# Ryannasr11/m2-tts

Hardware: AMD Instinct MI355X
Metric: audio samples/sec (22.05 kHz) + RTF, stage1_poc batch=32 @1/2/4/8 MI355X (higher is better)
Workload: dtype f32 (split 3xf16 MFMA, fp32 accumulate); 1 GPU; stage1_poc SimpleVocoder B=32 per GPU (configs[1]); stage=s1, per_gpu_batch=32, mel_frames=500, audio_samples_per_utt=32000, parallelism=weak-scaled replicas x1 (dp1, no collective in the data path)

## Files before the change

m2-tts_amd/csrc/m2_common.h:

```cpp
#pragma once

#include <hip/hip_runtime.h>
#include <stdint.h>
#include <string>

#include "../../include/m2tts_hip.h"

namespace m2 {

constexpr int kWave = 64;
constexpr float kLnEps = 1e-5f;
constexpr float kLeaky = 0.1f;
constexpr float kMaskFill = -1e9f;

enum Act : int { ACT_NONE = 0, ACT_LEAKY = 1, ACT_TANH = 2, ACT_RELU = 3, ACT_SOFTPLUS = 4 };

void set_error(const std::string& msg);

struct Switches {
    int dur_rb = 0;
    int dur_count = -1;
    int speculative = 1;
    bool tf_chain = true;
    bool tf_layer = true;
    bool tf_unfused = false;
    int tf_waves = 0;
    int tfl_rb = 0;
    int tfl_first_rb = 0;
    int tfl_rb_masked = 0;
    int tfl_rb_unmasked = 0;
    int tfl_qs2 = -1;
    int att_qt = 0;
    bool att_f32 = false;
    bool voc_perlayer = false;
    bool voc_f32 = false;
    bool voc_tail_x3 = false;
    bool voc_mid_x3 = false;
    int voc_plan = -1;
    int f32_mt = 2;
    bool f32_pair = true;
    int x3_head_prio = 0;
    bool f32_comp = true;
    int midp_nch = 0;
    int tailp_nch = 0;
    bool tailp_seven = false;
    int tailp2_nch = 0;
    bool tailp2_seven = false;
    bool head_inconv = false;
    int s2_mid_alt = -1;
    int s2_head_tf = 0;
    int redo_grid = -1;
    bool redo_launch = false;
    bool dur_split = true;
    bool dur_pers = true;
};
const Switches& sw();
void reload_switches();

int32_t fail(int32_t code, const char* what);
int32_t hip_status(hipError_t e, const char* where);

#define M2_CHECK_ARG(cond, msg)                      \
    do {                                             \
        if (!(cond)) return ::m2::fail(M2_E_ARG, msg); \
    } while (0)
#define M2_CHECK_SHAPE(cond, msg)                      \
    do {                                               \
        if (!(cond)) return ::m2::fail(M2_E_SHAPE, msg); \
    } while (0)
#define M2_HIP(expr)                                                   \
    do {                                                               \
        hipError_t _e = (expr);                                        \
        if (_e != hipSuccess) return ::m2::hip_status(_e, #expr);      \
    } while (0)
#define M2_LAUNCHED(name)                                              \
    do {                                                               \
        hipError_t _e = hipGetLastError();                             \
        if (_e != hipSuccess) return ::m2::hip_status(_e, name);       \
    } while (0)

__device__ __forceinline__ float apply_act(float v, int act) {
    if (act == ACT_LEAKY) return v > 0.f ? v : v * kLeaky;
    if (act == ACT_TANH) return tanhf(v);
    if (act == ACT_RELU) return v > 0.f ? v : 0.f;
    if (act == ACT_SOFTPLUS) return v > 20.f ? v : log1pf(expf(v));
    return v;
}

template <int ACT>
__device__ __forceinline__ float act_t(float v) {
    if constexpr (ACT == ACT_LEAKY) return fmaxf(v, v * kLeaky);
    else if constexpr (ACT == ACT_TANH) return tanhf(v);
    else if constexpr (ACT == ACT_RELU) return v > 0.f ? v : 0.f;
    else return v;
}

__device__ __forceinline__ int dev_frames(const int32_t* p, int cap) {
    const int t = max(1, *p);
    return t <= cap ? t : 0;
}

inline int cdiv(int a, int b) { return (a + b - 1) / b; }
inline size_t align_up(size_t v, size_t a) { return (v + a - 1) / a * a; }

struct Carve {
    char* base;
    size_t cap;
    size_t off = 0;
    bool ok = true;
    Carve(void* p, size_t n) : base(static_cast<char*>(p)), cap(n) {}
    template <typename T>
    T* take(size_t count) {
        size_t o = align_up(off, 256);
        size_t n = count * sizeof(T);
        if (o + n > cap || base == nullptr) { ok = false; off = o + n; return nullptr; }
        off = o + n;
        return reinterpret_cast<T*>(base + o);
    }
};

struct Sizer {
    size_t off = 0;
    template <typename T>
    T* take(size_t count) { off = align_up(off, 256) + count * sizeof(T); return nullptr; }
};

__device__ __forceinline__ void ln_row_stats(const float* xr, int K, int lane, float& mean, float& rstd) {
    float s = 0.f;
    for (int k = lane; k < K; k += 64) s = __fadd_rn(s, xr[k]);
    for (int o = 32; o > 0; o >>= 1) s = __fadd_rn(s, __shfl_xor(s, o));
    mean = __fdiv_rn(s, (float)K);
    float v = 0.f;
    for (int k = lane; k < K; k += 64) {
        const float d = __fsub_rn(xr[k], mean);
        v = __fmaf_rn(d, d, v);
    }
    for (int o = 32; o > 0; o >>= 1) v = __fadd_rn(v, __shfl_xor(v, o));
    rstd = __fdiv_rn(1.0f, __fsqrt_rn(__fadd_rn(__fdiv_rn(v, (float)K), kLnEps)));
}

template <int KP>
__device__ __forceinline__ void ln_row_stats_regs(const float (&x)[KP], int K, int lane, float& mean, float& rstd) {
    float s = 0.f;
#pragma unroll
    for (int q = 0; q < KP; ++q)
        if (lane + 64 * q < K) s = __fadd_rn(s, x[q]);
    for (int o = 32; o > 0; o >>= 1) s = __fadd_rn(s, __shfl_xor(s, o));
    mean = __fdiv_rn(s, (float)K);
    float v = 0.f;
#pragma unroll
    for (int q = 0; q < KP; ++q)
        if (lane + 64 * q < K) {
            const float d = __fsub_rn(x[q], mean);
            v = __fmaf_rn(d, d, v);
        }
    for (int o = 32; o > 0; o >>= 1) v = __fadd_rn(v, __shfl_xor(v, o));
    rstd = __fdiv_rn(1.0f, __fsqrt_rn(__fadd_rn(__fdiv_rn(v, (float)K), kLnEps)));
}

__device__ __forceinline__ float ln_apply(float x, float mean, float rstd, float g, float b) {
    return __fmaf_rn(__fmul_rn(__fsub_rn(x, mean), rstd), g, b);
}

}
```

m2-tts_amd/csrc/m2_runtime.hip:

```cpp
#include <immintrin.h>

#include <atomic>
#include <climits>
#include <cmath>
#include <cstdlib>
#include <cstring>
#include <mutex>
#include <new>
#include <string>
#include <vector>

#include "m2_common.h"
#include "m2_model.h"
#include "transformer_fused.h"
#include "transformer_layer.h"
#include "vocoder_fused.h"

namespace m2 {

namespace {
std::atomic<const Switches*> g_swp{nullptr};
std::mutex g_sw_mu;
int env_int(const char* name, int dflt) {
    const char* e = std::getenv(name);
    return (e && *e) ? std::atoi(e) : dflt;
}
bool env_set(const char* name) { return std::getenv(name) != nullptr; }
bool env_on(const char* name, bool dflt) {
    const char* e = std::getenv(name);
    return (e && *e) ? std::atoi(e) != 0 : dflt;
}
const bool g_sw_loaded = (reload_switches(), true);
}

const Switches& sw() { return *g_swp.load(std::memory_order_acquire); }

void reload_switches() {
    void* raw = std::calloc(1, sizeof(Switches));
    if (!raw) return;
    Switches& s = *new (raw) Switches();
    const int rb = env_int("M2_DUR_RB", 0);
    s.dur_rb = (rb == 1 || rb == 2) ? rb : 0;
    s.dur_count = std::getenv("M2_DUR_COUNT") && *std::getenv("M2_DUR_COUNT") ? (env_int("M2_DUR_COUNT", 0) != 0) : -1;
    s.speculative = env_on("M2_SPECULATIVE", true) ? 1 : 0;
    s.tf_chain = env_on("M2_TF_CHAIN", true);
    s.tf_layer = env_on("M2_TF_LAYER", true);
    s.tf_unfused = env_set("M2_TF_UNFUSED");
    const int tw = env_int("M2_TF_WAVES", 0);
    s.tf_waves = (tw == 4 || tw == 8) ? tw : 0;
    auto rb124 = [](int v) { return (v == 1 || v == 2 || v == 4) ? v : 0; };
    const int trb = env_int("M2_TFL_RB", 0);
    s.tfl_rb = rb124(trb);
    s.tfl_first_rb = rb124(env_int("M2_TFL_FIRST_RB", 0));
    s.tfl_rb_masked = rb124(env_int("M2_TFL_RB_MASKED", 0));
    s.tfl_rb_unmasked = rb124(env_int("M2_TFL_RB_UNMASKED", 0));
    if (const char* e = std::getenv("M2_TFL_QS2"); e && *e) {
        const int v = std::atoi(e);
        s.tfl_qs2 = (v == 2 || v == 3 || v == 4 || v == 12) ? v : 0;
    }
    s.att_qt = env_int("M2_ATT_QT", 0);
    if (const char* e = std::getenv("M2_ATT_F32")) s.att_f32 = *e && *e != '0';
    s.voc_perlayer = env_set("M2_VOCODER_PERLAYER");
    s.voc_f32 = env_set("M2_VOC_F32");
    s.voc_tail_x3 = env_set("M2_VOC_TAIL_X3");
    s.voc_mid_x3 = env_set("M2_VOC_MID_X3");
    s.voc_plan = env_int("M2_VOC_PLAN", -1);
    s.f32_mt = env_int("M2_F32_MT", 2);
    s.f32_pair = env_int("M2_F32_PAIR", 1) != 0;
    s.f32_comp = env_int("M2_F32_COMP", 1) != 0;
    s.x3_head_prio = env_int("M2_X3_HEAD_PRIO", 0);
    const int mn = env_int("M2_MIDP_NCH", 0);
    s.midp_nch = mn > 0 ? mn : 0;
    const int tn = env_int("M2_TAILP_NCH", 0);
    s.tailp_nch = tn > 0 ? tn : 0;
    s.tailp_seven = env_set("M2_TAILP_SEVEN");
    s.tailp2_nch = env_int("M2_TAILP2_NCH", 0);
    s.tailp2_seven = env_set("M2_TAILP2_SEVEN");
    s.head_inconv = env_set("M2_HEAD_INCONV");
    const int malt = env_int("M2_S2_MID_ALT", -1);
    s.s2_mid_alt = (malt == 0 || malt == 1) ? malt : -1;
    const int htf = env_int("M2_S2_HEAD_TF", env_set("M2_S2_HEAD_TF16") ? 16 : 0);
    s.s2_head_tf = (htf == 16 || htf == 19 || htf == 24 || htf == 27) ? htf : 0;
    s.redo_grid = env_int("M2_REDO_GRID", -1);
    s.redo_launch = env_set("M2_REDO_LAUNCH");
    s.dur_split = env_on("M2_DUR_SPLIT", true);
    s.dur_pers = env_on("M2_DUR_PERS", true);
    std::lock_guard<std::mutex> lk(g_sw_mu);
    const Switches* cur = g_swp.load(std::memory_order_relaxed);
    if (cur && std::memcmp(cur, &s, sizeof(Switches)) == 0) {
        std::free(raw);
        return;
    }
    g_swp.store(&s, std::memory_order_release);
}

int32_t launch_embed_pe(const int64_t*, const float*, const float*, int, int, int, int, float*, const int64_t*,
                        uint8_t*, hipStream_t);
int32_t launch_layer_norm(const float*, const float*, const float*, int, int, float*, hipStream_t);
int32_t launch_linear(const float*, const float*, const float*, const float*, const float*,
                      const float*, int, int, int, int, float*, hipStream_t);
int32_t launch_attention(const float*, const uint8_t*, int, int, int, int, float*, hipStream_t, bool force_f32 = false);
int32_t launch_duration(const float*, int, int, int, const float* const*, float*, hipStream_t,
                        const float* ln_g = nullptr, const float* ln_b = nullptr, float* enc_out = nullptr,
                        const float* const* wsplit = nullptr);
int32_t launch_duration_count(const float*, int, int, int, const float* const*, float*, hipStream_t, const float*,
                              const float*, float*, float, int32_t*, int32_t*, int32_t*, unsigned*, int32_t*, int32_t,
                              const float* const* wsplit = nullptr);
bool duration_count_fusable(int, int);
int32_t launch_lr_count(const void*, int, float, int, int, int32_t*, int32_t*, int32_t*, hipStream_t);
int32_t launch_lr_count_sync(const void*, int, float, int, int, int32_t*, int32_t*, int32_t*, unsigned*, int32_t*,
                             int32_t, hipStream_t);
int32_t launch_lr_expand(const float*, const int32_t*, int, int, int, int, float*, hipStream_t);
int32_t launch_conv(const float*, const float*, const float*, const float*, const float*,
                    const float*, int, int, bool, int, int, int, int, float*, hipStream_t);
int32_t launch_add_pe(const float*, const float*, int, int, int, float*, hipStream_t);
int32_t launch_embed_pe_scaled(const int64_t*, const float*, const float*, int, int, int, int, float, float*, hipStream_t);
int32_t launch_convT(const float*, const float*, const float*, int, int, int, int, int, int,
                     float*, hipStream_t);
int32_t launch_conv_general(const float*, const float*, const float*, const float*, const float*, const float*, int,
                            int, int, int, int, int, int, int, float*, hipStream_t);
int32_t launch_ragged_count(const int32_t*, int, int32_t*, hipStream_t);
int32_t launch_ragged_zero(float*, const int32_t*, int, int, int, hipStream_t);
int32_t launch_ragged_tail(const VocRedoW*, int, int, const float*, bool, const int32_t*, int, int, float*, hipStream_t);
int ragged_window_frames();
int32_t launch_ragged_gather(const float*, bool, const int32_t*, int, int, int, float*, hipStream_t);
int32_t launch_ragged_scatter(const float*, const int32_t*, int, int, float*, hipStream_t);

static thread_local std::string g_last_error;

void set_error(const std::string& msg) { g_last_error = msg; }

int32_t fail(int32_t code, const char* what) {
    set_error(what);
    return code;
}

int32_t hip_status(hipError_t e, const char* where) {
    set_error(std::string(where) + ": " + hipGetErrorString(e));
    return static_cast<int32_t>(e);
}

static constexpr int kVocHalo = 3;
static constexpr int32_t kMaxFrames = 1 << 24;

}

using namespace m2;

namespace {

int32_t mask_kernel_launch(const int64_t* lengths, int B, int S, uint8_t* mask, hipStream_t st);

__global__ void padding_mask_kernel(const int64_t* __restrict__ lengths, int B, int S,
                                    uint8_t* __restrict__ mask) {
    const int i = blockIdx.x * blockDim.x + threadIdx.x;
    if (i >= B * S) return;
    const int b = i / S, s = i - b * S;
    mask[i] = (int64_t)s < lengths[b] ? 1 : 0;
}

int32_t mask_kernel_launch(const int64_t* lengths, int B, int S, uint8_t* mask, hipStream_t st) {
    if (B * S == 0) return M2_OK;
    hipLaunchKernelGGL(padding_mask_kernel, dim3(cdiv(B * S, 256)), dim3(256), 0, st, lengths, B, S, mask);
    M2_LAUNCHED("padding_mask_kernel");
    return M2_OK;
}

struct TfBufs {
    float *x, *qkv, *att, *hid;
    uint8_t* mask;
    TflBufs tfl[2];
};

template <typename A>
void carve_tf(A& a, int B, int N, int H, int heads, TfBufs* out) {
    const size_t R = (size_t)B * N;
    float* x = a.template take<float>(R * H);
    uint8_t* mask = a.template take<uint8_t>(R);
    const size_t three = align_up(R * 3 * H * 4, 256) + align_up(R * H * 4, 256) + align_up(R * 2 * H * 4, 256);
    const size_t one = tfl_supported(H, heads) ? 2 * align_up(tfl_bytes(B, N, H, heads), 256) : 0;
    unsigned char* region = a.template take<unsigned char>(std::max(three, one));
    if (!out) return;
    *out = TfBufs{};
    out->x = x;
    out->mask = mask;
    if (!region) return;
    out->qkv = reinterpret_cast<float*>(region);
    out->att = reinterpret_cast<float*>(region + align_up(R * 3 * H * 4, 256));
    out->hid = reinterpret_cast<float*>(region + align_up(R * 3 * H * 4, 256) + align_up(R * H * 4, 256));
    if (one) {
        tfl_carve(region, B, N, H, heads, &out->tfl[0]);
        tfl_carve(region + align_up(tfl_bytes(B, N, H, heads), 256), B, N, H, heads, &out->tfl[1]);
    }
}

size_t vocoder_max_cl(const m2_config& c, int T) {
    size_t best = (size_t)c.vocoder_channels * T;
    size_t ch = c.vocoder_channels, L = T;
    for (int k = 0; k < 4; ++k) {
        ch /= 2;
        L *= kRates[k];
        best = std::max(best, ch * L);
    }
    return best;
}

template <typename A>
void carve_voc(A& a, const m2_config& c, int B, int T, float** bufs) {
    const size_t n = (size_t)B * vocoder_max_cl(c, T);
    for (int i = 0; i < 3; ++i) {
        float* p = a.template take<float>(n);
        if (bufs) bufs[i] = p;
    }
}

struct ChunkBufs {
    float *mel, *audio, *voc[3];
};

template <typename A>
void carve_chunked(A& a, const m2_config& c, int B, int T, int chunk, ChunkBufs* out) {
    const int W = std::min(T, chunk + 2 * kVocHalo);
    float* mel = a.template take<float>((size_t)B * c.mel_channels * W);
    float* audio = a.template take<float>((size_t)B * 64 * W);
    float* voc[3];
    carve_voc(a, c, B, W, voc);
    if (out) *out = ChunkBufs{mel, audio, {voc[0], voc[1], voc[2]}};
}

size_t vocoder_ws_bytes(const m2_model* m, int B, int T) {
    Sizer s;
    if (m->chunk_frames > 0 && T > m->chunk_frames) carve_chunked(s, m->cfg, B, T, m->chunk_frames, nullptr);
    else carve_voc(s, m->cfg, B, T, nullptr);
    return s.off;
}

struct FrontBufs {
    float *enc, *dur;
    int32_t *cum, *tot, *tmax;
    uint8_t* mask;
};

template <typename A>
void carve_front(A& a, int B, int S, int H, FrontBufs* out) {
    float* enc = a.template take<float>((size_t)B * S * H);
    float* dur = a.template take<float>((size_t)B * S);
    int32_t* cum = a.template take<int32_t>((size_t)B * (S + 1));
    int32_t* tot = a.template take<int32_t>((size_t)B);
    int32_t* tmax = a.template take<int32_t>(1);
    uint8_t* mask = a.template take<uint8_t>((size_t)B * S);
    if (out) *out = FrontBufs{enc, dur, cum, tot, tmax, mask};
}

int32_t run_layer(const m2_model* m, const m2_layer_w& L, const float* x_in, float* x, TfBufs& wb,
                  const uint8_t* mask, int B, int N, hipStream_t st) {
    const int H = m->cfg.hidden_dim, R = B * N;
    int32_t rc;
    if (m->tfused) {
        if ((rc = launch_ln_gemm(x_in, L.n1_w, L.n1_b, L.qkv_p, nullptr, ACT_NONE, R, H, 3 * H, wb.qkv, st))) return rc;
        if ((rc = launch_attention(wb.qkv, mask, B, N, H, m->cfg.num_heads, wb.att, st, m->att_f32))) return rc;
        return launch_post_attn(wb.att, x_in, L.out_p, L.out_b, L.n2_w, L.n2_b, L.ff1_p, L.ff1_b, L.ff2_p, L.ff2_b, R, H,
                                x, st);
    }
    if ((rc = launch_linear(x_in, L.n1_w, L.n1_b, L.qkv_w, nullptr, nullptr, ACT_NONE, R, H, 3 * H, wb.qkv, st))) return rc;
    if ((rc = launch_attention(wb.qkv, mask, B, N, H, m->cfg.num_heads, wb.att, st, m->att_f32))) return rc;
    if ((rc = launch_linear(wb.att, nullptr, nullptr, L.out_w, L.out_b, x_in, ACT_NONE, R, H, H, x, st))) return rc;
    if ((rc = launch_linear(x, L.n2_w, L.n2_b, L.ff1_w, L.ff1_b, nullptr, ACT_RELU, R, H, 2 * H, wb.hid, st))) return rc;
    if ((rc = launch_linear(wb.hid, nullptr, nullptr, L.ff2_w, L.ff2_b, x, ACT_NONE, R, 2 * H, H, x, st))) return rc;
    return M2_OK;
}

bool tf_chain(const m2_model* m) {
    const int H = m->cfg.hidden_dim;
    return sw().tf_chain && m->tfused && tf_post_next_supported(H, 3 * H);
}

bool tf_first_fused(const m2_model* m, const std::vector<m2_layer_w>& layers) {
    return tf_chain(m) && !layers.empty() && tf_src_fused_supported(m->cfg.hidden_dim, 3 * m->cfg.hidden_dim);
}

TflQueue tfl_queue(const m2_model* m) { return TflQueue{m->tflq, m->tfl_seq++}; }
int32_t tfl_reset(const m2_model* m, hipStream_t st, int32_t rc) {
    (void)hipMemsetAsync(m->tflq, 0, kTflQueueWords * sizeof(unsigned), st);
    m->tfl_seq = 0;
    return rc;
}

bool tfl_use(const m2_model* m, const std::vector<m2_layer_w>& layers) {
    return sw().tf_layer && m->tfused && !m->att_f32 && !layers.empty() &&
           tfl_supported(m->cfg.hidden_dim, m->cfg.num_heads);
}

int32_t run_tfl(const m2_model* m, const std::vector<m2_layer_w>& layers, const float* x0, float* x, TfBufs& wb,
                const int64_t* lengths, int B, int N, hipStream_t st, const float* fin_g = nullptr,
                const float* fin_b = nullptr, const float* fin_W = nullptr, const float* fin_bias = nullptr,
                int fin_N = 0, float* fin_out = nullptr, bool* fin_done = nullptr, const int32_t* dN = nullptr,
                const int32_t* rows = nullptr) {
    const int H = m->cfg.hidden_dim, heads = m->cfg.num_heads, n = (int)layers.size();
    if (fin_done) *fin_done = false;
    const float* cur = x0;
    for (int l = 0; l < n; ++l) {
        const m2_layer_w& L = layers[l];
        TflLayer w{L.out_p, L.out_b, L.n2_w, L.n2_b, L.ff1_p, L.ff1_b, L.ff2_p, L.ff2_b};
        w.wide_scores = L.wide_scores;
        int next = 0, NN = 0;
        float* z = nullptr;
        if (l + 1 < n) {
            next = 1;
            w.gn = layers[l + 1].n1_w;
            w.bn = layers[l + 1].n1_b;
            w.Wn = layers[l + 1].qkv_p;
        } else if (fin_W && tfl_proj_supported(H, fin_N)) {
            next = 2;
            w.gn = fin_g;
            w.bn = fin_b;
            w.Wn = fin_W;
            w.bn2 = fin_bias;
            NN = fin_N;
            z = fin_out;
        }
        const int32_t rc = launch_tfl_layer(w, B, N, H, heads, lengths != nullptr, lengths, cur, x, wb.tfl[l & 1], next,
                                            wb.tfl[(l + 1) & 1], NN, z, tfl_queue(m), st, dN, rows);
        if (rc) return tfl_reset(m, st, rc);
        if (next == 2 && fin_done) *fin_done = true;
        cur = x;
    }
    return M2_OK;
}

int32_t run_stack(const m2_model* m, const std::vector<m2_layer_w>& layers, const float* x_in, float* x, TfBufs& wb,
                  const uint8_t* mask, int B, int N, hipStream_t st, const float* fin_g = nullptr,
                  const float* fin_b = nullptr, const float* fin_W = nullptr, const float* fin_bias = nullptr,
                  int fin_N = 0, float* fin_out = nullptr, bool* fin_done = nullptr, bool qkv_ready = false) {
    const int H = m->cfg.hidden_dim, R = B * N, n = (int)layers.size();
    if (fin_done) *fin_done = false;
    int32_t rc;
    const bool chain = tf_chain(m);
    if (!chain) {
        const float* cur = x_in;
        for (const auto& L : layers) {
            if ((rc = run_layer(m, L, cur, x, wb, mask, B, N, st))) return rc;
            cur = x;
        }
        return M2_OK;
    }
    if (n == 0) return M2_OK;
    const float* cur = x_in;
    if (!qkv_ready && (rc = launch_ln_gemm(cur, layers[0].n1_w, layers[0].n1_b, layers[0].qkv_p, nullptr, ACT_NONE, R,
                                           H, 3 * H, wb.qkv, st)))
        return rc;
    for (int l = 0; l < n; ++l) {
        const m2_layer_w& L = layers[l];
        if ((rc = launch_attention(wb.qkv, mask, B, N, H, m->cfg.num_heads, wb.att, st, m->att_f32))) return rc;
        if (l + 1 < n) {
            const m2_layer_w& Nx = layers[l + 1];
            rc = launch_post_attn_next(wb.att, cur, L.out_p, L.out_b, L.n2_w, L.n2_b, L.ff1_p, L.ff1_b, L.ff2_p,
                                       L.ff2_b, R, H, x, Nx.n1_w, Nx.n1_b, Nx.qkv_p, nullptr, 3 * H, wb.qkv, st);
        } else if (fin_W && tf_post_next_supported(H, fin_N)) {
            rc = launch_post_attn_next(wb.att, cur, L.out_p, L.out_b, L.n2_w, L.n2_b, L.ff1_p, L.ff1_b, L.ff2_p,
                                       L.ff2_b, R, H, x, fin_g, fin_b, fin_W, fin_bias, fin_N, fin_out, st);
            if (!rc && fin_done) *fin_done = true;
        } else {
            rc = launch_post_attn(wb.att, cur, L.out_p, L.out_b, L.n2_w, L.n2_b, L.ff1_p, L.ff1_b, L.ff2_p, L.ff2_b, R,
                                  H, x, st);
        }
        if (rc) return rc;
        cur = x;
    }
    return M2_OK;
}

}

extern "C" {

int32_t m2_abi_version(void) { return M2_ABI_VERSION; }

const char* m2_last_error(void) { return g_last_error.c_str(); }
// ... 962 lines not shown
```

m2-tts_amd/csrc/vocoder_tailp.hip:

```cpp
#include <algorithm>
#include <cstdlib>
#include <vector>

#include "m2_common.h"
#include "vocoder_fused.h"
#include "vocoder_pipe.h"

namespace m2 {
namespace tp {

using namespace pipe;

constexpr int kRingRows[7] = {64, 64, 64, 64, 64, 64, 48};
constexpr int kRingOff(int n) { return n == 0 ? 0 : kRingOff(n - 1) + kRingRows[n - 1] * 128; }
constexpr int kLoOff(int n) { return kRingRows[n] * 64; }
constexpr int kPeriod(int n) { return kRingRows[n] / 16; }
constexpr int kCorrSlot = kRingOff(6);
constexpr int ring_bytes(int nl) { return nl == 6 ? kCorrSlot + 16 : kRingOff(nl); }
constexpr int kFlagOff(int nl) { return ring_bytes(nl); }
constexpr int lds_bytes(int nl) { return ring_bytes(nl) + 16; }
constexpr int nwaves(int nl) { return nl + 1; }
static_assert(lds_bytes(6) * 3 <= 160 * 1024, "three workgroups per CU");
static_assert(lds_bytes(7) * 2 <= 160 * 1024, "two workgroups per CU");
#ifdef M2_STAMPS
constexpr int NWAVES = 8;
#endif

__device__ __forceinline__ unsigned ring_at(int n, int row, int oct) {
    return kRingOff(n) + row * 64 + 16 * (oct ^ ((row >> 1) & 3));
}

#ifdef M2_STAMPS
__device__ unsigned long long g_tp_stamps[1024][NWAVES][64][2];
#define TPSTAMP(i, j)                                                                                  \
    do {                                                                                               \
        __builtin_amdgcn_sched_barrier(0);                                                             \
        unsigned long long _t;                                                                         \
        asm volatile("s_memtime %0\n\ts_waitcnt lgkmcnt(0)" : "=s"(_t)::"memory");                    \
        __builtin_amdgcn_sched_barrier(0);                                                             \
        const int _wg = blockIdx.y * gridDim.x + blockIdx.x;                                           \
        if ((threadIdx.x & 63) == 0 && _wg < 1024 && (i) < 64) g_tp_stamps[_wg][threadIdx.x >> 6][(i)][(j)] = _t; \
    } while (0)
#else
#define TPSTAMP(i, j) \
    do {              \
    } while (0)
#endif

template <int L, int NMB, int NL>
__device__ __forceinline__ void layer_role(unsigned char* lds, int qa, int L2, int nch, bool edge,
                                           const u32x4* __restrict__ W, const float* __restrict__ bias,
                                           float* __restrict__ arow, int* rflag) {
    constexpr int NKB = nkb(L), NF = nfrag(L);
    constexpr bool RES = L == 2 || L == 5;
    constexpr int ACT = RES ? ACT_NONE : ACT_LEAKY;
    const int lane = threadIdx.x & 63, li = lane & 15, g = lane >> 4;
    auto used = [](int f) {
        bool u = false;
        for (int m = 0; m < NMB; ++m)
            for (int kb = 0; kb < nkbm(L, m); ++kb) u = u || frag(L, m, kb) == f;
        return u;
    };
    u32x4 a[NMB][NKB][2];
    float bv[NMB][4];
#pragma unroll
    for (int m = 0; m < NMB; ++m) {
#pragma unroll
        for (int kb = 0; kb < nkbm(L, m); ++kb) {
            const int u = unit0(L) + m * NKB + kb;
            a[m][kb][0] = W[u * 128 + lane];
            a[m][kb][1] = W[u * 128 + 64 + lane];
        }
#pragma unroll
        for (int r = 0; r < 4; ++r) bv[m][r] = bias[L * 32 + m * 16 + 4 * g + r];
    }
    constexpr int PI = kPeriod(L), PO = L < 6 ? kPeriod(L + 1) : 1, PX = RES ? kPeriod(L - 1) : 1;
    unsigned radr[NF][PI], xadr[PX], oadr[PO];
#pragma unroll
    for (int j = 0; j < PI; ++j)
#pragma unroll
        for (int f = 0; f < NF; ++f) {
            const Slot sl = fslot(L, f, g);
            radr[f][j] = ring_at(L, ring_row(kRingRows[L], j, li + sl.dq - 1), sl.oct);
        }
#pragma unroll
    for (int j = 0; j < PX; ++j) xadr[j] = RES ? ring_at(L - 1, ring_row(kRingRows[L - 1], j, li - 2), g) : 0u;
    constexpr unsigned MX = L == 3 ? 16u : 32u;
    const int obase = L == 3 ? 1 + (g >> 1) : (g >> 1);
#pragma unroll
    for (int j = 0; j < PO; ++j)
        oadr[j] = L < 6 ? (g & 1) * kLoOff(L + 1) + ring_at(L + 1, ring_row(kRingRows[L + 1], j, li), obase) : 0u;
    u32x4 aid[NMB];
#pragma unroll
    for (int m = 0; m < NMB; ++m) {
        h8 v;
#pragma unroll
        for (int e = 0; e < 8; ++e) v[e] = (_Float16)(16 * m + li == 8 * g + e ? 1.f : 0.f);
        aid[m] = __builtin_bit_cast(u32x4, v);
    }
    const int sL = qa + NL - 1 - L;
    auto work = [&](int k, auto jc) {
        constexpr int kk = decltype(jc)::value;
        constexpr int ji = kk % PI, jx = kk % PX, jo = kk % PO;
        u32x4 bh[NF], bl[NF];
#pragma unroll
        for (int f = 0; f < NF; ++f)
            if (used(f)) {
                bh[f] = *reinterpret_cast<const u32x4*>(lds + radr[f][ji]);
                bl[f] = *reinterpret_cast<const u32x4*>(lds + radr[f][ji] + kLoOff(L));
            }
        u32x4 xh, xl;
        if constexpr (RES) {
            xh = *reinterpret_cast<const u32x4*>(lds + xadr[jx]);
            xl = *reinterpret_cast<const u32x4*>(lds + xadr[jx] + kLoOff(L - 1));
        }
        f32x4 acc[NMB];
#pragma unroll
        for (int m = 0; m < NMB; ++m) acc[m] = f32x4{bv[m][0], bv[m][1], bv[m][2], bv[m][3]};
#pragma unroll
        for (int kb = 0; kb < NKB; ++kb)
#pragma unroll
            for (int pr = 0; pr < 3; ++pr)
#pragma unroll
                for (int m = 0; m < NMB; ++m)
                    if (kb < nkbm(L, m)) {
                        const int f = frag(L, m, kb);
                        acc[m] = mfma_h(a[m][kb][pr == 2], pr == 1 ? bl[f] : bh[f], acc[m]);
                    }
        if constexpr (RES) {
#pragma unroll
            for (int m = 0; m < NMB; ++m) acc[m] = mfma_h(aid[m], xh, acc[m]);
#pragma unroll
            for (int m = 0; m < NMB; ++m) acc[m] = mfma_h(aid[m], xl, acc[m]);
        }
        const int x0 = sL + 16 * k;
        if constexpr (L == NL - 1) {
            const int x = x0 + li;
            if (g == 0 && k >= 0 && x >= 0 && x < L2) {
                float4 o;
                o.x = tanh_fast(acc[0][0]);
                o.y = tanh_fast(acc[0][1]);
                o.z = tanh_fast(acc[0][2]);
                o.w = tanh_fast(acc[0][3]);
                *reinterpret_cast<float4*>(arow + 4 * (size_t)x) = o;
                flag_nonfinite4(o.x, o.y, o.z, o.w, rflag, reinterpret_cast<int*>(lds + kFlagOff(NL)));
            }
        } else {
            auto epilogue = [&](auto zc) {
                constexpr bool ZERO = decltype(zc)::value;
                float v[NMB][4];
#pragma unroll
                for (int m = 0; m < NMB; ++m) {
#pragma unroll
                    for (int r = 0; r < 4; ++r) v[m][r] = acc[m][r];
                    if constexpr (ACT == ACT_LEAKY) leaky4(v[m]);
                }
                if constexpr (ZERO) {
                    const int x = x0 + li;
                    const bool out = x < 0 || x >= L2;
#pragma unroll
                    for (int m = 0; m < NMB; ++m)
#pragma unroll
                        for (int r = 0; r < 4; ++r) v[m][r] = out ? 0.f : v[m][r];
                    if constexpr (L == 4 && NL == 6) {
                        const float* cp = bias + kOutcCorr;
                        asm volatile("" : "+s"(cp));
                        const bool right = g >= 2;
                        if (right ? x == L2 - 1 : x == 0) {
                            const float* cv = cp + (right ? 8 + 4 * (g - 2) : 4 * g);
                            float d = g == 0 ? cp[16] : (g == 2 ? cp[17] : 0.f);
#pragma unroll
                            for (int r = 0; r < 4; ++r) d = fmaf(cv[r], right ? v[1][r] : v[0][r], d);
                            *reinterpret_cast<float*>(lds + kCorrSlot + 4 * g) = d;
                        }
                    }
                }
#pragma unroll
                for (int m = 0; m < NMB; ++m) {
                    unsigned h0, h1, l0, l1;
                    split2u(v[m][0], v[m][1], h0, l0);
                    split2u(v[m][2], v[m][3], h1, l1);
                    const auto s0 = __builtin_amdgcn_permlane16_swap(h0, l0, false, false);
                    const auto s1 = __builtin_amdgcn_permlane16_swap(h1, l1, false, false);
                    *reinterpret_cast<u32x4*>(lds + (oadr[jo] ^ (MX * m))) = u32x4{s0[0], s1[0], s0[1], s1[1]};
                }
            };
            constexpr int EW = L == 4 && NL == 6 ? 1 : 0;
            if (edge && (x0 < EW || x0 + 16 > L2 - EW)) epilogue(std::true_type{});
            else epilogue(std::false_type{});
        }
    };
    const int LAST = last_step(nch, NL);
    auto step = [&](int s, auto jc) {
        if (s <= LAST) {
            TPSTAMP(s + 1, 0);
            const int k = s - off_l(L);
            if (k >= -1 && k < nch) work(k, jc);
            TPSTAMP(s + 1, 1);
            step_barrier();
        }
    };
    constexpr int U = (PI == 3 || PO == 3 || PX == 3) ? 12 : 4;
    constexpr int J0 = ((-1 - off_l(L)) % U + U) % U;
    auto iter = [&](int s, auto... i) { (step(s + decltype(i)::value, ic<(J0 + decltype(i)::value) % U>{}), ...); };
#pragma unroll 1
    for (int s = -1; s <= LAST; s += U) {
        if constexpr (U == 4)
            iter(s, ic<0>{}, ic<1>{}, ic<2>{}, ic<3>{});
        else
            iter(s, ic<0>{}, ic<1>{}, ic<2>{}, ic<3>{}, ic<4>{}, ic<5>{}, ic<6>{}, ic<7>{}, ic<8>{}, ic<9>{},
                 ic<10>{}, ic<11>{});
    }
}

__device__ __forceinline__ void outc_role(unsigned char* lds, int qa, int L2, int nch, bool edge,
                                          const u32x4* __restrict__ W, const float* __restrict__ bias,
                                          float* __restrict__ arow, int* rflag) {
    constexpr int L = 5, NL = 6, NF = 4, P = 4;
    const int lane = threadIdx.x & 63, li = lane & 15, g = lane >> 4;
    u32x4 a[NF][2];
#pragma unroll
    for (int f = 0; f < NF; ++f) {
        a[f][0] = W[(kOutcUnit0 + f) * 128 + lane];
        a[f][1] = W[(kOutcUnit0 + f) * 128 + 64 + lane];
    }
    float bv[4];
#pragma unroll
    for (int r = 0; r < 4; ++r) bv[r] = bias[kOutcBias + 4 * g + r];
    static_assert(kRingRows[4] == 64 && kRingRows[5] == 64, "64-row rings");
    unsigned rbase[NF];
#pragma unroll
    for (int f = 0; f < NF; ++f) {
        const Slot sl = outc_slot(f, g);
        rbase[f] = f < 2 ? ring_at(5, ring_row(kRingRows[5], 0, li + sl.dq - 1), sl.oct) - kRingOff(5)
                         : ring_at(4, ring_row(kRingRows[4], 0, li + sl.dq - 2), sl.oct) - kRingOff(4);
    }
    auto radr = [&](int f, int j) { return (f < 2 ? kRingOff(5) : kRingOff(4)) + ((rbase[f] + 1024u * j) & 4095u); };
    auto work = [&](int k, auto jc) {
        constexpr int j = decltype(jc)::value;
        u32x4 bh[NF], bl[NF];
#pragma unroll
        for (int f = 0; f < NF; ++f) {
            bh[f] = *reinterpret_cast<const u32x4*>(lds + radr(f, j));
            bl[f] = *reinterpret_cast<const u32x4*>(lds + radr(f, j) + (f < 2 ? kLoOff(5) : kLoOff(4)));
        }
        const int x0 = qa + 16 * k, x = x0 + li;
        f32x4 acc = f32x4{bv[0], bv[1], bv[2], bv[3]};
#pragma unroll
        for (int f = 0; f < NF; ++f)
#pragma unroll
            for (int pr = 0; pr < 3; ++pr) acc = mfma_h(a[f][pr == 2], pr == 1 ? bl[f] : bh[f], acc);
        float v[4] = {acc[0], acc[1], acc[2], acc[3]};
        if (edge && (x0 <= 0 || x0 + 16 >= L2)) {
            const f32x4 e = *reinterpret_cast<const f32x4*>(lds + kCorrSlot);
            if (x == 0) v[0] -= e[0] + e[1];
            if (x == L2 - 1) v[3] -= e[2] + e[3];
        }
        if (g == 0 && k >= 0 && x >= 0 && x < L2) {
            float4 o;
            o.x = tanh_fast(v[0]);
            o.y = tanh_fast(v[1]);
            o.z = tanh_fast(v[2]);
            o.w = tanh_fast(v[3]);
            *reinterpret_cast<float4*>(arow + 4 * (size_t)x) = o;
            flag_nonfinite4(o.x, o.y, o.z, o.w, rflag, reinterpret_cast<int*>(lds + kFlagOff(NL)));
        }
    };
    const int LAST = last_step(nch, NL);
    auto step = [&](int s, auto jc) {
        if (s <= LAST) {
            const int k = s - off_l(L);
            if (k >= 0 && k < nch) work(k, jc);
            step_barrier();
        }
    };
    constexpr int J0 = ((-1 - off_l(L)) % P + P) % P;
#pragma unroll 1
    for (int s = -1; s <= LAST; s += P) {
        step(s, ic<J0 % P>{});
        step(s + 1, ic<(J0 + 1) % P>{});
        step(s + 2, ic<(J0 + 2) % P>{});
        step(s + 3, ic<(J0 + 3) % P>{});
    }
}

template <int NL>
__device__ __forceinline__ void loader_role_dma(unsigned char* lds, int qa, int L2, int nch,
                                                const unsigned char* __restrict__ u2) {
    static_assert(NL > 0 && kRingRows[0] == 64, "4-chunk R0");
    const int lane = threadIdx.x & 63, row = lane >> 2;
    [[maybe_unused]] const int oct = (lane & 3) ^ ((row >> 1) & 3);
    const int c0 = max(0, qa + NL - 16);
    [[maybe_unused]] const auto rs = __builtin_amdgcn_make_buffer_rsrc(
        const_cast<unsigned char*>(u2) + (size_t)c0 * 128, 0, (int)min((long)(L2 - c0) * 128, 0x7fffffffL),
        0x00020000);
    auto dma = [&](int c) {
#if defined(__HIP_DEVICE_COMPILE__)
        const int voff = (qa + NL + 16 * c + row - c0) * 128 + 16 * oct;
        unsigned char* dst = lds + kRingOff(0) + 1024 * (c & 3);
        __builtin_amdgcn_raw_ptr_buffer_load_lds(rs, (__attribute__((address_space(3))) void*)dst, 16, voff, 0, 0,
                                                 0);
        __builtin_amdgcn_raw_ptr_buffer_load_lds(rs, (__attribute__((address_space(3))) void*)(dst + kLoOff(0)), 16,
                                                 voff + 64, 0, 0, 0);
#endif
    };
    dma(-1);
#pragma unroll 1
    for (int s = -1; s <= last_step(nch, NL); ++s) {
        if (s + 1 < nch) {
            dma(s + 1);
            asm volatile("s_waitcnt vmcnt(2)" ::: "memory");
        } else {
            asm volatile("s_waitcnt vmcnt(0)" ::: "memory");
        }
        step_barrier();
    }
}

template <int NL, int NCHC>
__global__ __launch_bounds__(nwaves(NL) * 64, 6) void tailp_kernel(const unsigned char* __restrict__ U2, int L2,
                                                                    int nch_arg, const u32x4* __restrict__ W,
                                                                    const float* __restrict__ bias,
                                                                    float* __restrict__ audio, int* rflag,
                                                                    const int32_t* __restrict__ dT, VocRedo rd) {
    extern __shared__ __attribute__((aligned(16))) unsigned char lds[];
    const int nch = NCHC ? NCHC : nch_arg;
    const int b = blockIdx.y, qa = blockIdx.x * 16 * nch;
    if (dT) {
        L2 = 16 * dev_frames(dT, L2 / 16);
        if (qa >= L2) return;
    }
    const int w = __builtin_amdgcn_readfirstlane(threadIdx.x >> 6);
    const bool edge = qa < 32 || qa + 16 * nch + 32 > L2;
    float* arow = audio + (size_t)b * 4 * L2;
    int* const lflag = reinterpret_cast<int*>(lds + kFlagOff(NL));
    if (threadIdx.x == 0) *lflag = 0;
    TPSTAMP(62, 0);
    if (w >= 5) __builtin_amdgcn_s_setprio(3);
    else if (w >= 3) __builtin_amdgcn_s_setprio(2);
    else if (w >= 1) __builtin_amdgcn_s_setprio(1);
    const unsigned char* u2 = U2 + (size_t)b * L2 * 128;
    switch (w) {
        case 0: layer_role<0, 2, NL>(lds, qa, L2, nch, edge, W, bias, arow, rflag); break;
        case 1: layer_role<1, 2, NL>(lds, qa, L2, nch, edge, W, bias, arow, rflag); break;
        case 2: layer_role<2, 2, NL>(lds, qa, L2, nch, edge, W, bias, arow, rflag); break;
        case 3: layer_role<3, 2, NL>(lds, qa, L2, nch, edge, W, bias, arow, rflag); break;
        case 4: layer_role<4, 2, NL>(lds, qa, L2, nch, edge, W, bias, arow, rflag); break;
        case 5:
            if constexpr (NL == 7) layer_role<5, 2, NL>(lds, qa, L2, nch, edge, W, bias, arow, rflag);
            else outc_role(lds, qa, L2, nch, edge, W, bias, arow, rflag);
            break;
        case 6:
            if constexpr (NL == 7) {
                layer_role<6, 1, NL>(lds, qa, L2, nch, edge, W, bias, arow, rflag);
                break;
            }
            [[fallthrough]];
        default:
            loader_role_dma<NL>(lds, qa, L2, nch, u2);
            break;
    }
    TPSTAMP(63, 0);
    if (rd.rw) {
        __syncthreads();
        if (*lflag)
            redo_frames(*rd.rw, rd.mel, rd.trans, L2 / 16, b, qa / 16, min(L2, qa + 16 * nch) / 16, arow,
                        reinterpret_cast<float*>(lds), ring_bytes(NL) / 4);
    }
}

template <int NL, int NCHC>
int32_t launch(int nch, const void* U2, int L2, int B, const vx_u32x4* W, const float* bias, float* audio,
               int* rflag, hipStream_t st, const int32_t* dT, const VocRedo& rd) {
    static bool attr = false;
    if (!attr) {
        M2_HIP(hipFuncSetAttribute(reinterpret_cast<const void*>(tailp_kernel<NL, NCHC>),
                                   hipFuncAttributeMaxDynamicSharedMemorySize, lds_bytes(NL)));
        attr = true;
    }
    hipLaunchKernelGGL((tailp_kernel<NL, NCHC>), dim3(cdiv(L2, 16 * nch), B), dim3(nwaves(NL) * 64), lds_bytes(NL),
                       st, static_cast<const unsigned char*>(U2), L2, nch, W, bias, audio, rflag, dT, rd);
    M2_LAUNCHED("tailp_kernel");
    return M2_OK;
}
template <int NL>
int32_t launch_nl(int nch, const void* U2, int L2, int B, const vx_u32x4* W, const float* bias, float* audio,
                  int* rflag, hipStream_t st, const int32_t* dT, const VocRedo& rd) {
    return nch == 21 ? launch<NL, 21>(nch, U2, L2, B, W, bias, audio, rflag, st, dT, rd)
                     : launch<NL, 0>(nch, U2, L2, B, W, bias, audio, rflag, st, dT, rd);
}

}

#ifdef M2_STAMPS
extern "C" int32_t m2_debug_stamps_tailp(void* host, size_t bytes) {
    return (int32_t)hipMemcpyFromSymbol(host, HIP_SYMBOL(tp::g_tp_stamps),
                                        bytes < sizeof(tp::g_tp_stamps) ? bytes : sizeof(tp::g_tp_stamps));
}
#endif

const char* const kVocTailpKernelName =
    "tailp_kernel (ConvT3 + ResBlock3 + ConvT4 + ResBlock4 + output_conv, pipelined)";

int32_t launch_vocoder_tailp(const void* U2, int L2, int B, const vx_u32x4* W, const float* bias, float* audio,
                             int* rflag, hipStream_t st, const int32_t* dT, const VocRedo& rd) {
    if (B == 0 || L2 == 0) return M2_OK;
    const int nl = sw().tailp_seven ? 7 : 6;
    int nch = sw().tailp_nch > 0 ? std::min(sw().tailp_nch, 4096) : 0;
    if (!nch) nch = pipe::pick_strip(cdiv(L2, 16), B, 8, 768, nl + 1);
    const bool seven = sw().tailp_seven;
    return seven ? tp::launch_nl<7>(nch, U2, L2, B, W, bias, audio, rflag, st, dT, rd)
                 : tp::launch_nl<6>(nch, U2, L2, B, W, bias, audio, rflag, st, dT, rd);
}

bool pack_tailp(const TailpSrc& s, std::vector<uint16_t>* wout, std::vector<float>* bout, bool* range_ok) {
    using namespace pipe;
    const int nrows[tp::kLayers] = {32, 32, 32, 32, 32, 32, 4};
    std::vector<PolyDense> d;
    for (int l = 0; l < tp::kLayers; ++l) d.emplace_back(nrows[l], 32);
    dense_convT2(d[0], s.wt3, 1, 32, 16);
    dense_conv3(d[1], s.w31, 2, 16, 16);
    dense_conv3(d[2], s.w32, 2, 16, 16);
    dense_convT2(d[3], s.wt4, 2, 16, 8);
    dense_conv3(d[4], s.w41, 4, 8, 8);
    dense_conv3(d[5], s.w42, 4, 8, 8);
    dense_conv3(d[6], s.wo, 4, 8, 1);
    wout->assign((size_t)(tp::kUnits + tp::kOutcUnits) * 2 * 64 * 8, 0);
    for (int l = 0; l < tp::kLayers; ++l)
        for (int mb = 0; mb < tp::nmb(l); ++mb)
            if (!cut_fragments(
                    d[l], tp::unit0(l) + mb * tp::nkb(l), tp::nkbm(l, mb),
                    [&](int li) { return tp::prow(l, mb * 16 + li); },
                    [&](int kb, int g) { return tp::kslot(l, mb, kb, g); }, wout, range_ok))
                return false;
    bout->assign(tp::kBiasFloats, 0.f);
    const float* bsrc[tp::kLayers] = {s.bt3, s.b31, s.b32, s.bt4, s.b41, s.b42, s.bo};
    const int cper[tp::kLayers] = {16, 16, 16, 8, 8, 8, 1};
    for (int l = 0; l < tp::kLayers; ++l)
        for (int R = 0; R < nrows[l]; ++R) (*bout)[l * 32 + R] = bsrc[l][tp::prow(l, R) % cper[l]];
    return pack_outc_layer(s, 8, tp::kOutcUnit0, 2, 2, tp::outc_slot, tp::kOutcBias, tp::kOutcCorr, wout, bout,
                           range_ok);
}

}
```

Baseline: 15.62 billion audio samples/s.

## Fold tailp loader wave into layer-0 wave via async buffer-to-LDS DMA

By default the dedicated loader wave in the pipelined vocoder tail kernel is removed. The layer-0 compute wave now issues the buffer_load_lds prefetch for the next chunk itself and waits on vmcnt before the step barrier. Dropping one wave per workgroup should cut barrier participants and per-CU wave pressure. It also adds sched_barrier bursts and asm register pins to keep weights resident in registers. The risk is that layer 0 may stall on DMA latency, which lengthens the critical pipeline stage; the old loader wave can be restored with an environment variable.

Result: no change. 15.74 billion audio samples/s, median of 6 (+0.8%).

```diff
diff --git a/m2-tts_amd/csrc/m2_common.h b/m2-tts_amd/csrc/m2_common.h
--- a/m2-tts_amd/csrc/m2_common.h
+++ b/m2-tts_amd/csrc/m2_common.h
@@ -44,6 +44,7 @@
     int midp_nch = 0;
     int tailp_nch = 0;
     bool tailp_seven = false;
+    int pipe_loader_wave = 0;
     int tailp2_nch = 0;
     bool tailp2_seven = false;
     bool head_inconv = false;
diff --git a/m2-tts_amd/csrc/m2_runtime.hip b/m2-tts_amd/csrc/m2_runtime.hip
--- a/m2-tts_amd/csrc/m2_runtime.hip
+++ b/m2-tts_amd/csrc/m2_runtime.hip
@@ -74,6 +74,8 @@
     const int tn = env_int("M2_TAILP_NCH", 0);
     s.tailp_nch = tn > 0 ? tn : 0;
     s.tailp_seven = env_set("M2_TAILP_SEVEN");
+    if (const char* e = std::getenv("M2_PIPE_LOADER_WAVE"); e && *e)
+        s.pipe_loader_wave = (e[1] == 0 && (*e == '0' || *e == '1')) ? *e - '0' : -1;
     s.tailp2_nch = env_int("M2_TAILP2_NCH", 0);
     s.tailp2_seven = env_set("M2_TAILP2_SEVEN");
     s.head_inconv = env_set("M2_HEAD_INCONV");
diff --git a/m2-tts_amd/csrc/vocoder_tailp.hip b/m2-tts_amd/csrc/vocoder_tailp.hip
--- a/m2-tts_amd/csrc/vocoder_tailp.hip
+++ b/m2-tts_amd/csrc/vocoder_tailp.hip
@@ -19,7 +19,11 @@
 constexpr int ring_bytes(int nl) { return nl == 6 ? kCorrSlot + 16 : kRingOff(nl); }
 constexpr int kFlagOff(int nl) { return ring_bytes(nl); }
 constexpr int lds_bytes(int nl) { return ring_bytes(nl) + 16; }
-constexpr int nwaves(int nl) { return nl + 1; }
+constexpr int nwaves(int nl, bool lw) { return nl + (lw ? 1 : 0); }
+constexpr int kWavesPerSimd = 6;
+#ifndef TAILP_BURST
+#define TAILP_BURST 1
+#endif
 static_assert(lds_bytes(6) * 3 <= 160 * 1024, "three workgroups per CU");
 static_assert(lds_bytes(7) * 2 <= 160 * 1024, "two workgroups per CU");
 #ifdef M2_STAMPS
@@ -47,12 +51,41 @@
     } while (0)
 #endif
 
-template <int L, int NMB, int NL>
+template <int NL>
+__device__ __forceinline__ auto r0_dma(unsigned char* lds, int qa, int L2, const unsigned char* __restrict__ u2) {
+    static_assert(NL > 0 && kRingRows[0] == 64, "4-chunk R0");
+    const int lane = threadIdx.x & 63, row = lane >> 2;
+    const int oct = (lane & 3) ^ ((row >> 1) & 3);
+    const int c0 = max(0, qa + NL - 16);
+    [[maybe_unused]] const auto rs = __builtin_amdgcn_make_buffer_rsrc(
+        const_cast<unsigned char*>(u2) + (size_t)c0 * 128, 0, (int)min((long)(L2 - c0) * 128, 0x7fffffffL),
+        0x00020000);
+    [[maybe_unused]] const int voff0 = (qa + NL + row - c0) * 128 + 16 * oct;
+    return [=]([[maybe_unused]] int c) {
+#if defined(__HIP_DEVICE_COMPILE__)
+        const int voff = voff0 + 2048 * c;
+        unsigned char* dst = lds + kRingOff(0) + 1024 * (c & 3);
+        __builtin_amdgcn_raw_ptr_buffer_load_lds(rs, (__attribute__((address_space(3))) void*)dst, 16, voff, 0, 0,
+                                                 0);
+        __builtin_amdgcn_raw_ptr_buffer_load_lds(rs, (__attribute__((address_space(3))) void*)(dst + kLoOff(0)), 16,
+                                                 voff + 64, 0, 0, 0);
+#endif
+    };
+}
+__device__ __forceinline__ void dma_wait(bool issued) {
+    if (issued) asm volatile("s_waitcnt vmcnt(2)" ::: "memory");
+    else asm volatile("s_waitcnt vmcnt(0)" ::: "memory");
+}
+
+template <int L, int NMB, int NL, bool LW>
 __device__ __forceinline__ void layer_role(unsigned char* lds, int qa, int L2, int nch, bool edge,
                                            const u32x4* __restrict__ W, const float* __restrict__ bias,
-                                           float* __restrict__ arow, int* rflag) {
+                                           float* __restrict__ arow, int* rflag,
+                                           const unsigned char* __restrict__ u2) {
     constexpr int NKB = nkb(L), NF = nfrag(L);
     constexpr bool RES = L == 2 || L == 5;
+    constexpr bool DMA = L == 0 && !LW, BURST = !LW && TAILP_BURST && !RES;
+    const auto dma = r0_dma<NL>(lds, qa, L2, u2);
     constexpr int ACT = RES ? ACT_NONE : ACT_LEAKY;
     const int lane = threadIdx.x & 63, li = lane & 15, g = lane >> 4;
     auto used = [](int f) {
@@ -73,6 +106,15 @@
         }
 #pragma unroll
         for (int r = 0; r < 4; ++r) bv[m][r] = bias[L * 32 + m * 16 + 4 * g + r];
+    }
+    if constexpr (!LW) {
+#pragma unroll
+        for (int m = 0; m < NMB; ++m) {
+#pragma unroll
+            for (int kb = 0; kb < nkbm(L, m); ++kb) asm volatile("" ::"v"(a[m][kb][0]), "v"(a[m][kb][1]));
+#pragma unroll
+            for (int r = 0; r < 4; ++r) asm volatile("" ::"v"(bv[m][r]));
+        }
     }
     constexpr int PI = kPeriod(L), PO = L < 6 ? kPeriod(L + 1) : 1, PX = RES ? kPeriod(L - 1) : 1;
     unsigned radr[NF][PI], xadr[PX], oadr[PO];
@@ -114,6 +156,7 @@
             xh = *reinterpret_cast<const u32x4*>(lds + xadr[jx]);
             xl = *reinterpret_cast<const u32x4*>(lds + xadr[jx] + kLoOff(L - 1));
         }
+        if constexpr (BURST) __builtin_amdgcn_sched_barrier(0);
         f32x4 acc[NMB];
 #pragma unroll
         for (int m = 0; m < NMB; ++m) acc[m] = f32x4{bv[m][0], bv[m][1], bv[m][2], bv[m][3]};
@@ -194,12 +237,16 @@
     auto step = [&](int s, auto jc) {
         if (s <= LAST) {
             TPSTAMP(s + 1, 0);
+            if constexpr (DMA)
+                if (s + 1 < nch) dma(s + 1);
             const int k = s - off_l(L);
             if (k >= -1 && k < nch) work(k, jc);
             TPSTAMP(s + 1, 1);
+            if constexpr (DMA) dma_wait(s + 1 < nch);
             step_barrier();
         }
     };
+    if constexpr (DMA) dma(-1);
     constexpr int U = (PI == 3 || PO == 3 || PX == 3) ? 12 : 4;
     constexpr int J0 = ((-1 - off_l(L)) % U + U) % U;
     auto iter = [&](int s, auto... i) { (step(s + decltype(i)::value, ic<(J0 + decltype(i)::value) % U>{}), ...); };
@@ -213,6 +260,7 @@
     }
 }
 
+template <bool LW>
 __device__ __forceinline__ void outc_role(unsigned char* lds, int qa, int L2, int nch, bool edge,
                                           const u32x4* __restrict__ W, const float* __restrict__ bias,
                                           float* __restrict__ arow, int* rflag) {
@@ -227,6 +275,12 @@
     float bv[4];
 #pragma unroll
     for (int r = 0; r < 4; ++r) bv[r] = bias[kOutcBias + 4 * g + r];
+    if constexpr (!LW) {
+#pragma unroll
+        for (int f = 0; f < NF; ++f) asm volatile("" ::"v"(a[f][0]), "v"(a[f][1]));
+#pragma unroll
+        for (int r = 0; r < 4; ++r) asm volatile("" ::"v"(bv[r]));
+    }
     static_assert(kRingRows[4] == 64 && kRingRows[5] == 64, "64-row rings");
     unsigned rbase[NF];
 #pragma unroll
@@ -317,12 +371,11 @@
     }
 }
 
-template <int NL, int NCHC>
-__global__ __launch_bounds__(nwaves(NL) * 64, 6) void tailp_kernel(const unsigned char* __restrict__ U2, int L2,
-                                                                    int nch_arg, const u32x4* __restrict__ W,
-                                                                    const float* __restrict__ bias,
-                                                                    float* __restrict__ audio, int* rflag,
-                                                                    const int32_t* __restrict__ dT, VocRedo rd) {
+template <int NL, int NCHC, bool LW>
+__global__ __launch_bounds__(nwaves(NL, LW) * 64, kWavesPerSimd) void tailp_kernel(
+    const unsigned char* __restrict__ U2, int L2, int nch_arg, const u32x4* __restrict__ W,
+    const float* __restrict__ bias, float* __restrict__ audio, int* rflag, const int32_t* __restrict__ dT,
+    VocRedo rd) {
     extern __shared__ __attribute__((aligned(16))) unsigned char lds[];
     const int nch = NCHC ? NCHC : nch_arg;
     const int b = blockIdx.y, qa = blockIdx.x * 16 * nch;
@@ -341,23 +394,23 @@
     else if (w >= 1) __builtin_amdgcn_s_setprio(1);
     const unsigned char* u2 = U2 + (size_t)b * L2 * 128;
     switch (w) {
-        case 0: layer_role<0, 2, NL>(lds, qa, L2, nch, edge, W, bias, arow, rflag); break;
-        case 1: layer_role<1, 2, NL>(lds, qa, L2, nch, edge, W, bias, arow, rflag); break;
-        case 2: layer_role<2, 2, NL>(lds, qa, L2, nch, edge, W, bias, arow, rflag); break;
-        case 3: layer_role<3, 2, NL>(lds, qa, L2, nch, edge, W, bias, arow, rflag); break;
-        case 4: layer_role<4, 2, NL>(lds, qa, L2, nch, edge, W, bias, arow, rflag); break;
+        case 0: layer_role<0, 2, NL, LW>(lds, qa, L2, nch, edge, W, bias, arow, rflag, u2); break;
+        case 1: layer_role<1, 2, NL, LW>(lds, qa, L2, nch, edge, W, bias, arow, rflag, u2); break;
+        case 2: layer_role<2, 2, NL, LW>(lds, qa, L2, nch, edge, W, bias, arow, rflag, u2); break;
+        case 3: layer_role<3, 2, NL, LW>(lds, qa, L2, nch, edge, W, bias, arow, rflag, u2); break;
+        case 4: layer_role<4, 2, NL, LW>(lds, qa, L2, nch, edge, W, bias, arow, rflag, u2); break;
         case 5:
-            if constexpr (NL == 7) layer_role<5, 2, NL>(lds, qa, L2, nch, edge, W, bias, arow, rflag);
-            else outc_role(lds, qa, L2, nch, edge, W, bias, arow, rflag);
+            if constexpr (NL == 7) layer_role<5, 2, NL, LW>(lds, qa, L2, nch, edge, W, bias, arow, rflag, u2);
+            else outc_role<LW>(lds, qa, L2, nch, edge, W, bias, arow, rflag);
             break;
         case 6:
             if constexpr (NL == 7) {
-                layer_role<6, 1, NL>(lds, qa, L2, nch, edge, W, bias, arow, rflag);
+                layer_role<6, 1, NL, LW>(lds, qa, L2, nch, edge, W, bias, arow, rflag, u2);
                 break;
             }
             [[fallthrough]];
         default:
-            loader_role_dma<NL>(lds, qa, L2, nch, u2);
+            if constexpr (LW) loader_role_dma<NL>(lds, qa, L2, nch, u2);
             break;
     }
     TPSTAMP(63, 0);
@@ -369,25 +422,25 @@
     }
 }
 
-template <int NL, int NCHC>
+template <int NL, int NCHC, bool LW>
 int32_t launch(int nch, const void* U2, int L2, int B, const vx_u32x4* W, const float* bias, float* audio,
                int* rflag, hipStream_t st, const int32_t* dT, const VocRedo& rd) {
     static bool attr = false;
     if (!attr) {
-        M2_HIP(hipFuncSetAttribute(reinterpret_cast<const void*>(tailp_kernel<NL, NCHC>),
+        M2_HIP(hipFuncSetAttribute(reinterpret_cast<const void*>(tailp_kernel<NL, NCHC, LW>),
                                    hipFuncAttributeMaxDynamicSharedMemorySize, lds_bytes(NL)));
         attr = true;
     }
-    hipLaunchKernelGGL((tailp_kernel<NL, NCHC>), dim3(cdiv(L2, 16 * nch), B), dim3(nwaves(NL) * 64), lds_bytes(NL),
+    hipLaunchKernelGGL((tailp_kernel<NL, NCHC, LW>), dim3(cdiv(L2, 16 * nch), B), dim3(nwaves(NL, LW) * 64), lds_bytes(NL),
                        st, static_cast<const unsigned char*>(U2), L2, nch, W, bias, audio, rflag, dT, rd);
     M2_LAUNCHED("tailp_kernel");
     return M2_OK;
 }
-template <int NL>
+template <int NL, bool LW>
 int32_t launch_nl(int nch, const void* U2, int L2, int B, const vx_u32x4* W, const float* bias, float* audio,
                   int* rflag, hipStream_t st, const int32_t* dT, const VocRedo& rd) {
-    return nch == 21 ? launch<NL, 21>(nch, U2, L2, B, W, bias, audio, rflag, st, dT, rd)
-                     : launch<NL, 0>(nch, U2, L2, B, W, bias, audio, rflag, st, dT, rd);
+    return nch == 21 ? launch<NL, 21, LW>(nch, U2, L2, B, W, bias, audio, rflag, st, dT, rd)
+                     : launch<NL, 0, LW>(nch, U2, L2, B, W, bias, audio, rflag, st, dT, rd);
 }
 
 }
@@ -409,8 +462,13 @@
     int nch = sw().tailp_nch > 0 ? std::min(sw().tailp_nch, 4096) : 0;
     if (!nch) nch = pipe::pick_strip(cdiv(L2, 16), B, 8, 768, nl + 1);
     const bool seven = sw().tailp_seven;
-    return seven ? tp::launch_nl<7>(nch, U2, L2, B, W, bias, audio, rflag, st, dT, rd)
-                 : tp::launch_nl<6>(nch, U2, L2, B, W, bias, audio, rflag, st, dT, rd);
+    const int lw = sw().pipe_loader_wave;
+    if (lw != 0 && lw != 1) return fail(M2_E_ARG, "M2_PIPE_LOADER_WAVE: expected 0 or 1");
+    if (lw)
+        return seven ? tp::launch_nl<7, true>(nch, U2, L2, B, W, bias, audio, rflag, st, dT, rd)
+                     : tp::launch_nl<6, true>(nch, U2, L2, B, W, bias, audio, rflag, st, dT, rd);
+    return seven ? tp::launch_nl<7, false>(nch, U2, L2, B, W, bias, audio, rflag, st, dT, rd)
+                 : tp::launch_nl<6, false>(nch, U2, L2, B, W, bias, audio, rflag, st, dT, rd);
 }
 
 bool pack_tailp(const TailpSrc& s, std::vector<uint16_t>* wout, std::vector<float>* bout, bool* range_ok) {
```
